# valette/FROG

Hardware: AMD Instinct MI355X
Metric: registration iterations/sec (linear+deformable) (higher is better)
Workload: dtype f32

## Files before the change

frog_amd/_abi.py:

```python
import ctypes as C
import os

_HERE = os.path.dirname(os.path.abspath(__file__))
LIB_DIR = os.path.join(_HERE, "lib")



def usable_cpus():
    import math
    n = len(os.sched_getaffinity(0)) if hasattr(os, "sched_getaffinity") else (os.cpu_count() or 1)

    def quota(d):
        try:
            with open(os.path.join(d, "cpu.max")) as fh:
                q, p = fh.read().split()[:2]
            return None if q == "max" else float(q) / float(p)
        except (OSError, ValueError):
            pass
        try:
            with open(os.path.join(d, "cpu.cfs_quota_us")) as fh:
                q = float(fh.read())
            with open(os.path.join(d, "cpu.cfs_period_us")) as fh:
                p = float(fh.read())
            return q / p if q > 0 and p > 0 else None
# ... 322 lines not shown
    "frog_labels_fused": (C.c_int, [C.c_void_p, C.POINTER(FrogVolume), c_float_p]),
    "frog_labels_probability": (C.c_int, [C.c_void_p, C.c_int64, c_float_p]),
    "frog_labels_destroy": (None, [C.c_void_p]),
    "frog_staple_create": (C.c_int, [C.POINTER(FrogVolume), C.c_uint32, C.c_uint32, C.c_int, C.POINTER(C.c_void_p)]),
    "frog_staple_add": (C.c_int, [C.c_void_p, C.c_void_p, C.POINTER(FrogVolume), C.c_double, C.POINTER(FrogVolume)]),
    "frog_staple_finish": (C.c_int, [C.c_void_p, c_u32_p]),
    "frog_staple_values": (C.c_int, [C.c_void_p, C.POINTER(C.c_int64)]),
    "frog_staple_solve": (C.c_int, [C.c_void_p, C.c_double, C.c_double, C.c_uint32, C.c_int, c_u32_p, c_double_p,
                                    C.POINTER(C.c_uint64)]),
    "frog_staple_fused": (C.c_int, [C.c_void_p, C.POINTER(FrogVolume), c_float_p]),
    "frog_staple_probability": (C.c_int, [C.c_void_p, C.c_int64, c_float_p]),
    "frog_staple_performance": (C.c_int, [C.c_void_p, c_double_p, C.POINTER(C.c_uint64), C.POINTER(C.c_uint64), c_double_p]),
    "frog_staple_destroy": (None, [C.c_void_p]),
    "frog_wlabels_create": (C.c_int, [C.POINTER(FrogVolume), C.c_uint32, C.c_uint32, C.c_uint32, C.c_uint32, C.c_float, C.c_int,
                                      C.POINTER(C.c_void_p)]),
    "frog_wlabels_target": (C.c_int, [C.c_void_p, C.c_void_p, C.POINTER(FrogVolume), C.c_int, C.c_double, C.POINTER(FrogVolume)]),
    "frog_wlabels_add": (C.c_int, [C.c_void_p, C.c_void_p, C.POINTER(FrogVolume), C.POINTER(FrogVolume), C.c_int, C.c_double,
                                   C.c_double, C.POINTER(FrogVolume), C.POINTER(FrogVolume)]),
    "frog_wlabels_finish": (C.c_int, [C.c_void_p, c_u32_p]),
    "frog_wlabels_values": (C.c_int, [C.c_void_p, C.POINTER(C.c_int64)]),
    "frog_wlabels_fused": (C.c_int, [C.c_void_p, C.c_int64, C.POINTER(FrogVolume), c_float_p]),
    "frog_wlabels_probability": (C.c_int, [C.c_void_p, C.c_int64, c_float_p]),
    "frog_wlabels_destroy": (None, [C.c_void_p]),
    "frog_jlabels_create": (C.c_int, [C.POINTER(FrogVolume), C.c_uint32, C.c_uint32, C.c_uint32, C.c_uint32, C.c_double, C.c_int, C.c_int,
                                      C.POINTER(C.c_void_p)]),
    "frog_jlabels_target": (C.c_int, [C.c_void_p, C.c_void_p, C.POINTER(FrogVolume), C.c_int, C.c_double, C.POINTER(FrogVolume)]),
    "frog_jlabels_add": (C.c_int, [C.c_void_p, C.c_void_p, C.POINTER(FrogVolume), C.POINTER(FrogVolume), C.c_int, C.c_double,
                                   C.c_double, C.POINTER(FrogVolume), C.POINTER(FrogVolume)]),
    "frog_jlabels_finish": (C.c_int, [C.c_void_p, c_u32_p]),
    "frog_jlabels_values": (C.c_int, [C.c_void_p, C.POINTER(C.c_int64)]),
    "frog_jlabels_fused": (C.c_int, [C.c_void_p, C.c_int64, C.POINTER(FrogVolume), c_float_p]),
    "frog_jlabels_probability": (C.c_int, [C.c_void_p, C.c_int64, c_float_p]),
    "frog_jlabels_weight": (C.c_int, [C.c_void_p, C.c_uint32, c_float_p]),
    "frog_jlabels_destroy": (None, [C.c_void_p]),
    "frog_distance_map": (C.c_int, [C.POINTER(FrogVolume), C.c_int64, C.c_int, C.c_int, c_u32_p]),
    "frog_surface_create": (C.c_int, [C.POINTER(FrogVolume), C.POINTER(C.c_int64), C.c_uint32, C.c_uint32, C.c_int,
                                      C.POINTER(C.c_void_p)]),
    "frog_surface_add": (C.c_int, [C.c_void_p, C.c_void_p, C.POINTER(FrogVolume), C.c_double, C.POINTER(FrogSurfaceRow)]),
    "frog_surface_destroy": (None, [C.c_void_p]),
    "frog_isosurface_create": (C.c_int, [C.POINTER(FrogVolume), C.c_int, C.c_double, C.c_int64, C.c_int, C.POINTER(C.c_void_p),
                                         c_u32_p, c_u32_p]),
    "frog_isosurface_apply": (C.c_int, [C.c_void_p, C.c_void_p]),
    "frog_isosurface_get": (C.c_int, [C.c_void_p, c_float_p, c_u32_p]),
    "frog_isosurface_destroy": (None, [C.c_void_p]),
    "frog_chain_apply_f32": (C.c_int, [C.c_void_p, c_float_p, c_float_p, C.c_size_t]),
    "frog_match_options_default": (None, [C.POINTER(FrogMatchOptions)]),
    "frog_matcher_create": (C.c_int, [C.POINTER(FrogKeypoints), C.c_uint32, C.c_int, C.POINTER(C.c_void_p)]),
    "frog_matcher_destroy": (None, [C.c_void_p]),
    "frog_matcher_run": (C.c_int, [C.c_void_p, C.POINTER(C.c_uint16), C.POINTER(C.c_uint16), C.c_size_t,
                                   C.POINTER(FrogMatchOptions), C.POINTER(C.c_uint64), C.POINTER(c_u32_p),
                                   C.POINTER(c_u32_p)]),
    "frog_match_free": (None, [C.c_void_p]),
    "frog_matcher_last_stats": (C.c_int, [C.c_void_p, c_double_p, c_double_p]),
    "frog_matcher_last_forms": (C.c_int, [C.c_void_p, C.POINTER(C.c_uint64)]),
    "frog_match_test_products": (C.c_int, [C.c_int, c_float_p, c_float_p, C.c_uint32, C.c_int, c_float_p, c_float_p]),
    "frog_get_points2_subset": (C.c_int, [C.c_void_p, C.POINTER(C.c_uint64), C.c_size_t, c_float_p]),
    "frog_set_hard_links": (C.c_int, [C.c_void_p, C.POINTER(C.c_uint64), C.POINTER(C.c_uint64), C.c_size_t, C.c_float]),
    "frog_residual_sums": (C.c_int, [C.c_void_p]),
    "frog_get_error_map": (C.c_int, [C.c_void_p, C.c_uint32, C.POINTER(FrogGridInfo), c_float_p, C.c_size_t]),
    "frog_comm_buffer": (C.c_int, [C.c_void_p, C.c_int, C.POINTER(C.c_void_p), C.POINTER(C.c_size_t),
                                   C.POINTER(C.c_size_t), C.POINTER(C.c_size_t)]),
    "frog_update_stats_local": (C.c_int, [C.c_void_p]),
    "frog_stats_publish": (C.c_int, [C.c_void_p]),
    "frog_transform_points_local": (C.c_int, [C.c_void_p, C.c_int]),
    "frog_linear_step_local": (C.c_int, [C.c_void_p]),
    "frog_energy_read": (C.c_int, [C.c_void_p, c_double_p, c_double_p]),
    "frog_bounds_local": (C.c_int, [C.c_void_p, c_double_p, c_double_p]),
    "frog_deformable_setup_bounds": (C.c_int, [C.c_void_p, C.c_int, c_double_p, c_double_p, C.POINTER(FrogGridInfo)]),
    "frog_deformable_phase_a": (C.c_int, [C.c_void_p, C.c_float]),
    "frog_deformable_phase_b": (C.c_int, [C.c_void_p]),
    "frog_deformable_phase_c": (C.c_int, [C.c_void_p, c_double_p]),
    "frog_get_stream": (C.c_int, [C.c_void_p, C.POINTER(C.c_void_p), C.POINTER(C.c_int)]),
    "frog_comm_unpack_slab": (C.c_int, [C.c_void_p, C.c_void_p, C.c_uint64, C.c_uint32, C.POINTER(C.c_uint64), C.c_uint32]),
    "frog_comm_mode": (C.c_int, [C.c_void_p, C.c_int]),
    "frog_create_seconds": (C.c_int, [C.c_void_p, c_double_p, C.POINTER(C.c_int)]),
    "frog_lattice_reallocations": (C.c_int, [C.c_void_p, C.POINTER(C.c_int)]),
    "frog_transform_points_slab": (C.c_int, [C.c_void_p, C.c_int, C.c_int, C.c_void_p, C.c_uint64, C.c_uint32]),
    "frog_comm_unpack_slab_step": (C.c_int, [C.c_void_p, C.c_void_p, C.c_uint64, C.c_uint32, C.POINTER(C.c_uint64), C.c_uint32, C.c_uint32]),
    "frog_step_finish": (C.c_int, [C.c_void_p, C.POINTER(C.c_double)]),
    "frog_step_speculate": (C.c_int, [C.c_void_p]),
    "frog_cull_stats": (C.c_int, [C.c_void_p, C.POINTER(C.c_uint64), C.POINTER(C.c_uint64), C.POINTER(C.c_uint64)]),
    "frog_cull_stats_linear": (C.c_int, [C.c_void_p, C.POINTER(C.c_uint64), C.POINTER(C.c_uint64), C.POINTER(C.c_uint64)]),
    "frog_test_stray_points": (C.c_int, [C.c_void_p, C.POINTER(C.c_uint64)]),
    "frog_test_cull_ranges": (C.c_int, [C.c_void_p, C.POINTER(C.c_uint64), C.POINTER(C.c_uint64)]),
    "frog_test_cull_steps": (C.c_int, [C.c_void_p, C.POINTER(C.c_uint64), C.POINTER(C.c_uint64)]),
    "frog_test_cull_readback": (C.c_int, [C.c_void_p, c_float_p, c_float_p, c_float_p, c_u32_p, c_float_p, c_u32_p]),
    "frog_test_em_refit": (C.c_int, [C.c_void_p, C.c_int]),
    "frog_test_ransac_candidates": (C.c_int, [C.POINTER(FrogModel), C.c_uint32, C.POINTER(FrogRansacOptions), c_double_p,
                                              C.POINTER(C.c_ubyte), C.c_size_t, C.POINTER(C.c_size_t)]),
    "frog_test_ransac_census": (C.c_int, [C.c_void_p, C.POINTER(FrogModel), C.c_uint32, c_double_p, C.c_size_t, C.c_float,
                                          c_u32_p]),
    "frog_test_inlier_probability": (C.c_int, [C.c_int, c_float_p, c_float_p, C.c_size_t, c_float_p, c_float_p]),
    "frog_test_inlier_weight_pair": (C.c_int, [C.c_int, c_float_p, c_float_p, C.c_float, c_float_p, C.c_size_t, c_float_p,
                                              C.POINTER(C.c_ubyte)]),
    "frog_test_bspline_weights": (C.c_int, [C.c_int, C.c_void_p, C.c_size_t, C.c_void_p]),
    "frog_profile_enable": (C.c_int, [C.c_void_p, C.c_int]),
    "frog_profile_read": (C.c_int, [C.c_void_p, C.POINTER(FrogKernelTime), C.c_int]),
}

HOST_SYMBOLS = {
    "frog_pairs_read": (C.c_void_p, [C.c_char_p, C.POINTER(C.c_int)]),
    "frog_pairs_write": (C.c_int, [C.c_void_p, C.c_char_p]),
    "frog_pairs_free": (None, [C.c_void_p]),
    "frog_pairs_model": (None, [C.c_void_p, C.POINTER(FrogModel)]),
    "frog_pairs_num_pairs": (C.c_uint64, [C.c_void_p]),
    "frog_pairs_num_points": (C.c_uint64, [C.c_void_p]),
    "frog_pairs_num_images": (C.c_uint32, [C.c_void_p]),
    "frog_pairs_num_blocks": (C.c_uint32, [C.c_void_p]),
    "frog_host_threads": (C.c_int, []),
    "frog_pairs_block": (C.c_int, [C.c_void_p, C.c_uint32, C.POINTER(C.c_uint16), C.POINTER(C.c_uint16),
                                   C.POINTER(C.c_uint32), C.POINTER(c_u32_p), C.POINTER(c_u32_p)]),
    "frog_pairs_from_arrays": (C.c_void_p, [C.c_uint32, c_u32_p, c_float_p, c_float_p, C.c_uint32,
                                            C.POINTER(C.c_uint16), C.POINTER(C.c_uint16),
                                            C.POINTER(C.c_uint64), c_u32_p, c_u32_p]),
    "frog_synth_defaults": (None, [C.POINTER(FrogSynthParams)]),
    "frog_synth_generate": (C.c_void_p, [C.POINTER(FrogSynthParams)]),
    "frog_pairs_append_points": (C.c_int, [C.c_void_p, C.c_uint32, c_float_p, C.c_uint32]),
    "frog_pairs_set_points": (C.c_int, [C.c_void_p, C.c_uint32, c_float_p]),
    "frog_volume_read": (C.c_void_p, [C.c_char_p, C.POINTER(C.c_int)]),
    "frog_volume_free": (None, [C.c_void_p]),
    "frog_volume_view": (None, [C.c_void_p, C.POINTER(FrogVolume)]),
    "frog_volume_range": (C.c_int, [C.POINTER(FrogVolume), c_double_p, c_double_p]),
    "frog_volume_write": (C.c_int, [C.c_char_p, C.POINTER(FrogVolume)]),
    "frog_bbox_grid": (C.c_int, [C.c_char_p, C.c_double, C.POINTER(FrogVolume)]),
    "frog_score_metrics_from": (C.c_int, [C.POINTER(FrogScoreSums), C.POINTER(C.c_uint64), C.c_uint32, C.POINTER(FrogScoreMetrics)]),
    "frog_keypoints_read": (C.c_void_p, [C.c_char_p, C.POINTER(C.c_int)]),
    "frog_keypoints_free": (None, [C.c_void_p]),
    "frog_keypoints_count": (C.c_uint32, [C.c_void_p]),
    "frog_keypoints_view": (None, [C.c_void_p, C.POINTER(FrogKeypoints)]),
    "frog_keypoints_select": (C.c_int, [C.c_void_p, c_u32_p, C.c_uint32]),
    "frog_keypoints_write": (C.c_int, [C.c_char_p, C.POINTER(FrogKeypoints)]),
    "frog_transform_read": (C.c_void_p, [C.c_char_p, C.POINTER(C.c_int)]),
    "frog_transform_free": (None, [C.c_void_p]),
    "frog_transform_num_links": (C.c_uint32, [C.c_void_p]),
    "frog_transform_links": (C.POINTER(FrogChainLink), [C.c_void_p]),
    "frog_volume_geometry": (C.c_int, [C.c_char_p, C.POINTER(C.c_uint32), c_double_p, c_double_p]),
    "frog_nifti_write": (C.c_int, [C.c_char_p, C.POINTER(C.c_uint32), c_double_p, c_double_p, C.c_uint32, c_float_p]),
    "frog_run_schedule": (C.c_int, [C.c_void_p, C.c_void_p, C.POINTER(FrogSchedulePlan), C.POINTER(FrogScheduleResult)]),
    "frog_mesh_read": (C.c_void_p, [C.c_char_p, C.POINTER(C.c_int)]),
    "frog_mesh_view": (None, [C.c_void_p, C.POINTER(FrogMesh)]),
    "frog_mesh_free": (None, [C.c_void_p]),
    "frog_mesh_write": (C.c_int, [C.c_char_p, C.POINTER(FrogMesh)]),
    "frog_mesh_last_error": (C.c_char_p, []),
}

COMM_SYMBOLS = {
    "frog_comm_create_rccl": (C.c_int, [C.c_int, C.POINTER(C.c_int), C.POINTER(C.c_void_p)]),
    "frog_comm_create_loopback": (C.c_int, [C.c_int, C.POINTER(C.c_void_p)]),
    "frog_comm_unique_id": (C.c_int, [C.POINTER(C.c_ubyte)]),
    "frog_comm_create_rank": (C.c_int, [C.c_int, C.c_int, C.POINTER(C.c_ubyte), C.c_int, C.POINTER(C.c_void_p)]),
    "frog_comm_create_shm": (C.c_int, [C.c_int, C.c_int, C.c_char_p, C.c_int, C.POINTER(C.c_void_p)]),
    "frog_comm_set_rows": (C.c_int, [C.c_void_p, C.POINTER(C.c_uint64)]),
    "frog_comm_destroy_all": (None, [C.c_int, C.POINTER(C.c_void_p)]),
    "frog_comm_bind": (C.c_int, [C.c_void_p, C.c_void_p, c_u32_p]),
    "frog_comm_all_gather_xyz2": (C.c_int, [C.c_void_p]),
    "frog_comm_slab": (C.c_int, [C.c_void_p, C.POINTER(C.c_void_p), C.POINTER(C.c_uint64)]),
    "frog_comm_all_gather_slab": (C.c_int, [C.c_void_p]),
    "frog_comm_gather_points": (C.c_int, [C.c_void_p, C.c_int, C.c_int, C.c_uint32]),
    "frog_comm_all_reduce": (C.c_int, [C.c_void_p, C.c_int]),
    "frog_comm_all_reduce_bounds": (C.c_int, [C.c_void_p, c_double_p, c_double_p]),
    "frog_comm_barrier": (C.c_int, [C.c_void_p]),
    "frog_comm_timing": (C.c_int, [C.c_void_p, C.c_int]),
    "frog_comm_timing_read": (C.c_int, [C.c_void_p, c_double_p, C.POINTER(C.c_uint64), C.POINTER(C.c_uint64)]),
}


# ... 53 lines not shown
```

frog_amd/csrc/device/frog_hip.hip:

```cpp

#include "ctx.h"
#include <hip/hip_ext.h>
#include "prep.h"
#include "k_links.hip.h"
#include "k_stats.hip.h"
#include "k_grid.hip.h"
#include "k_comm.hip.h"
#include "k_cull.hip.h"
#include "k_ransac.hip.h"
#include "k_reforder.hip.h"
#include "k_refchain.hip.h"
#include "similarity.h"

#include <atomic>
#include <chrono>
#include <cmath>
#include <cstdlib>
#include <cstring>
#include <random>
#include <limits>
#include <new>

namespace frog {
thread_local std::string g_last_error;
// ... 2421 lines not shown
}

int frog_test_inlier_probability(int device, const float em3[3], const float *d2, size_t n, float *fast, float *exact)
{
    if (!em3 || (n && (!d2 || !fast || !exact))) return fail(FROG_E_INVALID, "null argument");
    int ndev = 0;
    if (hipGetDeviceCount(&ndev) != hipSuccess || ndev < 1) return fail(FROG_E_NODEVICE, "no HIP device");
    if (device < 0 || device >= ndev) return fail(FROG_E_INVALID, "device index out of range");
    FROG_HIP_CHECK(hipSetDevice(device));
    if (!n) return FROG_OK;
    DevBuf<float> dd, df, de;
    FROG_HIP_CHECK(dd.alloc(n)); FROG_HIP_CHECK(df.alloc(n)); FROG_HIP_CHECK(de.alloc(n));
    FROG_HIP_CHECK(hipMemcpy(dd.p, d2, n * sizeof(float), hipMemcpyHostToDevice));
    test_probability_kernel<<<div_up(n, 256), 256>>>(make_float4(em3[0], em3[1], em3[2], 0.f), dd.p, n, df.p, de.p);
    FROG_HIP_CHECK(hipGetLastError());
    FROG_HIP_CHECK(hipMemcpy(fast, df.p, n * sizeof(float), hipMemcpyDeviceToHost));
    FROG_HIP_CHECK(hipMemcpy(exact, de.p, n * sizeof(float), hipMemcpyDeviceToHost));
    return FROG_OK;
}

__global__ void test_weight_pair_kernel(const float4 emA, const float4 emB, float threshold, const float *d2, size_t n, float *weight,
                                        unsigned char *form)
{
    const size_t i = (size_t)blockIdx.x * blockDim.x + threadIdx.x;
    if (i >= n) return;
    const float theta = threshold - THRESHOLD_BAND;
    const EmFast fA = em_fast_of(emA, theta);
    EmFast fB = em_fast_of(emB, theta);
    fB.lo = fmaxf(fB.lo, fA.lo); fB.hi = fminf(fB.hi, fA.hi);
    bool in_range;
    float w = inlier_weight_pair(d2[i], fA, fB, in_range);
    unsigned char f = 0;
    if (w < theta) f = 2;
    else if (!in_range) { w = fminf(inlier_probability(d2[i], em_derived_of(emA)), inlier_probability(d2[i], em_derived_of(emB))); f = 1; }
    weight[i] = w; form[i] = f;
}

int frog_test_inlier_weight_pair(int device, const float emA3[3], const float emB3[3], float threshold, const float *d2, size_t n,
                                 float *weight, unsigned char *form)
{
    if (!emA3 || !emB3 || (n && (!d2 || !weight || !form))) return fail(FROG_E_INVALID, "null argument");
    int ndev = 0;
    if (hipGetDeviceCount(&ndev) != hipSuccess || ndev < 1) return fail(FROG_E_NODEVICE, "no HIP device");
    if (device < 0 || device >= ndev) return fail(FROG_E_INVALID, "device index out of range");
    FROG_HIP_CHECK(hipSetDevice(device));
    if (!n) return FROG_OK;
    DevBuf<float> dd, dw; DevBuf<unsigned char> df;
    FROG_HIP_CHECK(dd.alloc(n)); FROG_HIP_CHECK(dw.alloc(n)); FROG_HIP_CHECK(df.alloc(n));
    FROG_HIP_CHECK(hipMemcpy(dd.p, d2, n * sizeof(float), hipMemcpyHostToDevice));
    test_weight_pair_kernel<<<div_up(n, 256), 256>>>(make_float4(emA3[0], emA3[1], emA3[2], 0.f), make_float4(emB3[0], emB3[1], emB3[2], 0.f),
                                                      threshold, dd.p, n, dw.p, df.p);
    FROG_HIP_CHECK(hipGetLastError());
    FROG_HIP_CHECK(hipMemcpy(weight, dw.p, n * sizeof(float), hipMemcpyDeviceToHost));
    FROG_HIP_CHECK(hipMemcpy(form, df.p, n, hipMemcpyDeviceToHost));
    return FROG_OK;
}

__global__ void test_weights_kernel(const double *f, size_t n, double *out)
{
    const size_t i = (size_t)blockIdx.x * blockDim.x + threadIdx.x;
    if (i >= n) return;
    double F[4];
    bspline_weights<double>(F, f[i]);
    for (int k = 0; k < 4; k++) out[4 * i + k] = F[k];
}

int frog_test_bspline_weights(int device, const double *f, size_t n, double *out4n)
{
    if (n && (!f || !out4n)) return fail(FROG_E_INVALID, "null argument");
    int ndev = 0;
    if (hipGetDeviceCount(&ndev) != hipSuccess || ndev < 1) return fail(FROG_E_NODEVICE, "no HIP device");
    if (device < 0 || device >= ndev) return fail(FROG_E_INVALID, "device index out of range");
    FROG_HIP_CHECK(hipSetDevice(device));
    if (!n) return FROG_OK;
    DevBuf<double> df, dw;
    FROG_HIP_CHECK(df.alloc(n)); FROG_HIP_CHECK(dw.alloc(4 * n));
    FROG_HIP_CHECK(hipMemcpy(df.p, f, n * sizeof(double), hipMemcpyHostToDevice));
    test_weights_kernel<<<div_up(n, 256), 256>>>(df.p, n, dw.p);
    FROG_HIP_CHECK(hipGetLastError());
    FROG_HIP_CHECK(hipMemcpy(out4n, dw.p, 4 * n * sizeof(double), hipMemcpyDeviceToHost));
    return FROG_OK;
}

int frog_test_cull_ranges(frog_ctx *ctx, uint64_t *ranges, uint64_t *with_election)
{
    CTX_GUARD(ctx);
    if (!ranges || !with_election) return fail(FROG_E_INVALID, "null output");
    *ranges = 0; *with_election = 0;
    if (ctx->cull_builds && ctx->act_cnt.n) {
        std::vector<uint32_t> h(ctx->act_cnt.n);
        FROG_HIP_CHECK(hipMemcpyAsync(h.data(), ctx->act_cnt.p, ctx->act_cnt.bytes(), hipMemcpyDeviceToHost, ctx->stream));
        FROG_HIP_CHECK(hipStreamSynchronize(ctx->stream));
        for (uint32_t v : h) {
            if (v & ~CULL_DUP_BIT) (*ranges)++;
            if (v & CULL_DUP_BIT) (*with_election)++;
        }
    }
    return FROG_OK;
}

int frog_test_cull_steps(frog_ctx *ctx, uint64_t *listed_steps, uint64_t *steps_with_election)
{
    CTX_GUARD(ctx);
    if (!listed_steps || !steps_with_election) return fail(FROG_E_INVALID, "null output");
    *listed_steps = 0; *steps_with_election = 0;
    if (ctx->cull_builds && ctx->act_cnt.n) {
        std::vector<uint32_t> h(ctx->act_cnt.n), bits(ctx->act_steps.n);
        FROG_HIP_CHECK(hipMemcpyAsync(h.data(), ctx->act_cnt.p, ctx->act_cnt.bytes(), hipMemcpyDeviceToHost, ctx->stream));
        FROG_HIP_CHECK(hipMemcpyAsync(bits.data(), ctx->act_steps.p, ctx->act_steps.bytes(), hipMemcpyDeviceToHost, ctx->stream));
        FROG_HIP_CHECK(hipStreamSynchronize(ctx->stream));
        for (uint32_t v : h) *listed_steps += ((v & ~CULL_DUP_BIT) + 63u) / 64u;
        for (uint32_t v : bits) *steps_with_election += (uint64_t)__builtin_popcount(v);
    }
    return FROG_OK;
}

int frog_test_cull_readback(frog_ctx *ctx, float *cut_now, float *cut_list, float *allow, uint32_t *state, float *disp_max, uint32_t *disp_n)
{
    CTX_GUARD(ctx);
    if (!ctx->cut_now.p || !ctx->cut_list.p || !ctx->disp_part.p || !ctx->cull_state.p || !ctx->disp_allow.p)
        return fail(FROG_E_STATE, "the context has no culling list (FROG_CULL=0, a threshold below 1e-3, or its buffers did not fit)");
    hipStream_t s = ctx->stream;
    const uint32_t n = (uint32_t)std::min<size_t>(ctx->disp_n, ctx->disp_part.n);
    std::vector<uint32_t> part(disp_max ? n : 0);
    if (cut_now) FROG_HIP_CHECK(hipMemcpyAsync(cut_now, ctx->cut_now.p, (size_t)ctx->nI * sizeof(float), hipMemcpyDeviceToHost, s));
    if (cut_list) FROG_HIP_CHECK(hipMemcpyAsync(cut_list, ctx->cut_list.p, (size_t)ctx->nI * sizeof(float), hipMemcpyDeviceToHost, s));
    if (allow) FROG_HIP_CHECK(hipMemcpyAsync(allow, ctx->disp_allow.p, sizeof(float), hipMemcpyDeviceToHost, s));
    if (state) FROG_HIP_CHECK(hipMemcpyAsync(state, ctx->cull_state.p, sizeof(uint32_t), hipMemcpyDeviceToHost, s));
    if (!part.empty()) FROG_HIP_CHECK(hipMemcpyAsync(part.data(), ctx->disp_part.p, part.size() * sizeof(uint32_t), hipMemcpyDeviceToHost, s));
    FROG_HIP_CHECK(hipStreamSynchronize(s));
    if (disp_max) {
        uint32_t m = 0;
        for (uint32_t v : part) m = std::max(m, v);
        std::memcpy(disp_max, &m, sizeof m);
    }
    if (disp_n) *disp_n = n;
    return FROG_OK;
}

int frog_test_stray_points(frog_ctx *ctx, uint64_t *n)
{
    CTX_GUARD(ctx);
    { const int rc_ = join_setup(ctx); if (rc_) return rc_; }
    if (!n) return fail(FROG_E_INVALID, "null output");
    unsigned int v = 0;
    FROG_HIP_CHECK(hipMemcpyAsync(&v, ctx->stray.p + 2, sizeof v, hipMemcpyDeviceToHost, ctx->stream));
    FROG_HIP_CHECK(hipStreamSynchronize(ctx->stream));
    *n = v;
    return FROG_OK;
}

int frog_test_em_refit(frog_ctx *ctx, int term_by_term)
{
    CTX_GUARD(ctx);
    const uint32_t nO = ctx->n_owned(), cap = (uint32_t)ctx->sample_cap;
    const int cur = ctx->sel_used;
    hipStream_t s = ctx->stream;
    if (term_by_term)
        em_kernel<<<nO, 256, 0, s>>>(ctx->samples.p, ctx->sample_count[cur].p, cap, ctx->ib, ctx->em.p,
                                     ctx->opt.stats_max_iterations, ctx->opt.stats_epsilon);
    else
        em_scan_kernel<<<nO, EM_THREADS, 0, s>>>(ctx->samples.p, ctx->sample_count[cur].p, cap, ctx->ib, ctx->em.p,
                                                 ctx->opt.stats_max_iterations, ctx->opt.stats_epsilon, nullptr);
    FROG_HIP_CHECK(hipGetLastError());
    return frog_stats_publish(ctx);
}
// ... 187 lines not shown
```

frog_amd/csrc/device/k_grid.hip.h:

```cpp
#pragma once

#include "ctx.h"

namespace frog {

struct GeomDev {
    int dims[3];
    int n_cp;
    double origin[3];
    double spacing[3];
    double inv_spacing[3];
    int brick;
    int nbricks[3];
    int n_bricks;
    int lat_sh;
    uint32_t lat_mask;
    size_t lat_blk, lat_img;
    uint32_t mask_words;
};

__device__ __forceinline__ bool lat_active(const uint32_t *mask, const GeomDev &g, uint32_t img, uint32_t node)
{
    return (mask[(size_t)img * g.mask_words + (node >> 5)] >> (node & 31u)) & 1u;
}
// ... 738 lines not shown
        o.z = (float)((double)in[2] + (double)disp[2] * 1.0);
        o.w = v.w;
        pos2[p] = P3{ o.x, o.y, o.z };
        if (apply) pos[p] = o;
        if (snap) {
            const P3 q = snap[p];
            const float ex = o.x - q.x, ey = o.y - q.y, ez = o.z - q.z;
            dmax = max(dmax, __float_as_uint(__builtin_sqrtf(ex * ex + ey * ey + ez * ez)) & 0x7FFFFFFFu);
        }
    }
    if (snap) {
        #pragma unroll
        for (int off = 32; off > 0; off >>= 1) dmax = max(dmax, (uint32_t)__shfl_xor((int)dmax, off, 64));
        if (lane == 0) {
            disp_part[bid] = dmax;
            if (!(__uint_as_float(dmax) <= *disp_allow)) atomicOr(cull_state, 1u);
        }
    }
}

#ifdef FROG_SCATTER_TRACE
__device__ unsigned long long g_scatter_trace[4 * 65536];
#endif
constexpr int BRICK_CP_MAX = 11;


struct ScatterEnergy {
    const double *partial;
    uint32_t n;
    double *block_sums;
    unsigned int *ticket;
    double *energy;
    const uint32_t *list_invalid;
    unsigned int *stray_next;
    unsigned int *stray_total;
};

__device__ __forceinline__ void scatter_energy_block(const ScatterEnergy &en, const uint32_t r, const int lane)
{
    const uint32_t per = (en.n + ENERGY_BLOCKS - 1) / ENERGY_BLOCKS;
    const uint32_t b = min(en.n, r * per), e = min(en.n, b + per);
    double a0 = 0, a1 = 0;
    for (uint32_t t = b + lane; t < e; t += 64) { a0 += en.partial[2 * (size_t)t]; a1 += en.partial[2 * (size_t)t + 1]; }
    #pragma unroll
    for (int off = 32; off > 0; off >>= 1) { a0 += __shfl_down(a0, off, 64); a1 += __shfl_down(a1, off, 64); }
    bool last = false;
    if (lane == 0) {
        __hip_atomic_store(&en.block_sums[2 * r], a0, __ATOMIC_RELAXED, __HIP_MEMORY_SCOPE_AGENT);
        __hip_atomic_store(&en.block_sums[2 * r + 1], a1, __ATOMIC_RELAXED, __HIP_MEMORY_SCOPE_AGENT);
        __threadfence();
        last = atomicAdd(en.ticket, 1u) == (unsigned int)ENERGY_BLOCKS - 1u;
    }
    if (!__builtin_amdgcn_readfirstlane((int)last)) return;
    __threadfence();
    const double v0 = __hip_atomic_load(&en.block_sums[lane], __ATOMIC_RELAXED, __HIP_MEMORY_SCOPE_AGENT);
    const double v1 = __hip_atomic_load(&en.block_sums[64 + lane], __ATOMIC_RELAXED, __HIP_MEMORY_SCOPE_AGENT);
    double s0 = 0, s1 = 0;
    #pragma unroll 1
    for (int k = 0; k < ENERGY_BLOCKS; k++) {
        const int i0 = 2 * k, i1 = 2 * k + 1;
        const double x = __shfl(i0 < 64 ? v0 : v1, i0 & 63, 64), y = __shfl(i1 < 64 ? v0 : v1, i1 & 63, 64);
        s0 += x; s1 += y;
    }
    if (lane == 0) {
        en.energy[0] = s0; en.energy[1] = s1; en.energy[2] = 0.0;
        en.energy[3] = en.list_invalid ? (double)en.list_invalid[0] : 0.0;
        *en.stray_next = 0u;
        *en.ticket = 0u;
    }
}

#ifndef FROG_SCATTER_QUADS
#define FROG_SCATTER_QUADS 1
#endif
constexpr int SC_AHEAD = 3, SC_RING = 4;
#if FROG_SCATTER_QUADS
constexpr int SC_PTS = 64 + 4;
#else
constexpr int SC_PTS = 64 + SC_AHEAD;
#endif
struct ScatterScratch {
    float wx[4][SC_PTS], wy[4][SC_PTS];
    float wz[4][SC_PTS];
    float4 sm[SC_PTS];
    int base[SC_PTS];
};
static_assert(offsetof(ScatterScratch, sm) % 16 == 0, "ScatterScratch::sm is read with ds_read_b128");

#define FROG_FMAC_DPP(D, S, Q) "v_fmac_f32_dpp %" #D ", %" #S ", %8 quad_perm:[" #Q "," #Q "," #Q "," #Q "] row_mask:0xf bank_mask:0xf\n\t"
#define FROG_FMAC4_DPP(Q) asm volatile("s_nop 1\n\t" FROG_FMAC_DPP(0, 4, Q) FROG_FMAC_DPP(1, 5, Q) FROG_FMAC_DPP(2, 6, Q) FROG_FMAC_DPP(3, 7, Q)      \
                              : "+v"(run.x), "+v"(run.y), "+v"(run.z), "+v"(run.w) : "v"(s.x), "v"(s.y), "v"(s.z), "v"(s.w), "v"(w))
template <int P> __device__ __forceinline__ void fmac4_quad_bcast(float4 &run, const float4 s, float w)
{
    static_assert(P >= 0 && P < 4, "quad lane");
    if constexpr (P == 0) FROG_FMAC4_DPP(0);
    if constexpr (P == 1) FROG_FMAC4_DPP(1);
    if constexpr (P == 2) FROG_FMAC4_DPP(2);
    if constexpr (P == 3) FROG_FMAC4_DPP(3);
}

__global__ __launch_bounds__(64) void scatter_kernel(const float4 *pos_b, const float4 *point_sums,
                                                     const float4 *group_sums, uint32_t own_points, uint32_t own_pt_begin,
                                                     const uint32_t *perm, const ScatterBlock *blocks, const uint32_t *n_blocks,
                                                     float4 *gradf, float4 *stage, unsigned int *stray, const GeomDev g,
                                                     const ScatterEnergy en)
{
    if (en.partial && blockIdx.x < (uint32_t)ENERGY_BLOCKS) {
        scatter_energy_block(en, blockIdx.x, threadIdx.x);
        return;
    }
    const uint32_t bid = blockIdx.x - (en.partial ? (uint32_t)ENERGY_BLOCKS : 0u);
#ifdef FROG_SCATTER_TRACE
    const unsigned long long trace_t0 = wall_clock64();
    unsigned tr_load = 0, tr_p1 = 0, tr_p2 = 0;
#endif
    const ScatterBlock blk = blocks[bid];
    if (bid >= *n_blocks) return;
    extern __shared__ float4 tile[];
    __shared__ ScatterScratch sc;
    const int lane = threadIdx.x;
    const int E = g.brick + 3;
    const int n_tile = E * E * E;

    const uint32_t s_last = blk.end - 1u;
    const auto load_index = [&](uint32_t s) -> uint32_t { return perm[min(s, s_last)]; };
    const auto load_point = [&](uint32_t p, uint32_t s, float4 (&part)[N_XCD], float4 &v) __attribute__((always_inline)) {
        if (group_sums) {
            const uint32_t li = p - own_pt_begin;
            #pragma unroll
            for (int q = 0; q < N_XCD; q++) part[q] = group_sums[group_sum_index(q, li, own_points)];
        } else {
            part[0] = point_sums[p];
        }
        v = pos_b[min(s, s_last)];
    };
    uint32_t p_cur = load_index(blk.begin + lane);
    uint32_t p_nxt = load_index(blk.begin + 64 + lane);
    float4 part_cur[N_XCD], v_cur;
    #pragma unroll
    for (int q = 1; q < N_XCD; q++) part_cur[q] = make_float4(0.f, 0.f, 0.f, 0.f);
    load_point(p_cur, blk.begin + lane, part_cur, v_cur);

    for (int k = lane; k < n_tile; k += 64) tile[k] = make_float4(0.f, 0.f, 0.f, 0.f);

    const uint32_t img = blk.key / g.n_bricks;
    uint32_t bidx = blk.key - img * g.n_bricks;
    const int bx = bidx % g.nbricks[0]; bidx /= g.nbricks[0];
    const int by = bidx % g.nbricks[1];
    const int bz = bidx / g.nbricks[1];
    const int cp0[3] = { bx * g.brick, by * g.brick, bz * g.brick };

    const int ti = lane & 3, tj = (lane >> 2) & 3, tk = lane >> 4;
    const int tap_off = ti + E * (tj + E * tk);
    __builtin_amdgcn_fence(__ATOMIC_RELEASE, "wavefront");
    __builtin_amdgcn_wave_barrier();

    float4 run = make_float4(0.f, 0.f, 0.f, 0.f);
    int run_base = -1;
    for (uint32_t batch = blk.begin; batch < blk.end; batch += 64) {
        const uint32_t p_far = load_index(batch + 128 + lane);
        float4 part_nxt[N_XCD], v_nxt;
        #pragma unroll
        for (int q = 1; q < N_XCD; q++) part_nxt[q] = make_float4(0.f, 0.f, 0.f, 0.f);
        load_point(p_nxt, batch + 64 + lane, part_nxt, v_nxt);
#ifdef FROG_SCATTER_TRACE
        const unsigned long long tb0 = wall_clock64();
        asm volatile("s_waitcnt vmcnt(10)" ::: "memory");
        const unsigned long long tb1 = wall_clock64();
#endif
        float wxy[16], wz[4], wx4[4], wy4[4];
        float4 sm = part_cur[0];
        int base = -1;
        if (batch + lane < blk.end) {
            if (group_sums) {
                #pragma unroll
                for (int q = 1; q < N_XCD; q++) { sm.x += part_cur[q].x; sm.y += part_cur[q].y; sm.z += part_cur[q].z; sm.w += part_cur[q].w; }
            }
            if (sm.w != 0.f) {
                const float in[3] = { v_cur.x, v_cur.y, v_cur.z };
                int ic[3]; float fr[3];
                scatter_cell(in, g, ic, fr);
                double F[4];
                float w12[12];
                #pragma unroll
                for (int ax = 0; ax < 3; ax++) {
                    bspline_weights(F, (double)fr[ax]);
                    #pragma unroll
                    for (int m = 0; m < 4; m++) w12[ax * 4 + m] = (float)F[m];
                }
                #pragma unroll
                for (int j = 0; j < 4; j++)
                    #pragma unroll
                    for (int i = 0; i < 4; i++) wxy[4 * j + i] = w12[i] * w12[4 + j];
                #pragma unroll
                for (int k = 0; k < 4; k++) { wz[k] = w12[8 + k]; wx4[k] = w12[k]; wy4[k] = w12[4 + k]; }
                const int lx = ic[0] - 1 - cp0[0], ly = ic[1] - 1 - cp0[1], lz = ic[2] - 1 - cp0[2];
                if (lx >= 0 && ly >= 0 && lz >= 0 && lx + 3 < E && ly + 3 < E && lz + 3 < E) {
                    base = lx + E * (ly + E * lz);
                } else {
                    atomicAdd(stray, 1u);
                    atomicAdd(en.stray_total, 1u);
                    for (int k = 0; k < 4; k++) for (int j = 0; j < 4; j++) for (int i = 0; i < 4; i++) {
                        const int gx = ic[0] - 1 + i, gy = ic[1] - 1 + j, gz = ic[2] - 1 + k;
                        if (gx < 0 || gy < 0 || gz < 0 || gx >= g.dims[0] || gy >= g.dims[1] || gz >= g.dims[2]) continue;
                        const float w = wxy[4 * j + i] * wz[k];
                        float *dst = reinterpret_cast<float *>(gradf + lat(g, img, (uint32_t)gx + (uint32_t)g.dims[0] * ((uint32_t)gy + (uint32_t)g.dims[1] * (uint32_t)gz)));
                        atomicAdd(dst + 0, w * sm.x); atomicAdd(dst + 1, w * sm.y);
                        atomicAdd(dst + 2, w * sm.z); atomicAdd(dst + 3, w * sm.w);
                    }
                }
            }
        }
        const unsigned long long live = __ballot(base >= 0);
        const int n_live = __popcll(live);
        if (base >= 0) {
            const int slot = __popcll(live & ((1ull << lane) - 1ull));
            #pragma unroll
            for (int k = 0; k < 4; k++) { sc.wx[k][slot] = wx4[k]; sc.wy[k][slot] = wy4[k]; }
            #pragma unroll
            for (int k = 0; k < 4; k++) sc.wz[k][slot] = wz[k];
            sc.sm[slot] = sm;
            sc.base[slot] = base;
        }
        __builtin_amdgcn_fence(__ATOMIC_RELEASE, "wavefront");
        __builtin_amdgcn_wave_barrier();
#ifdef FROG_SCATTER_TRACE
        const unsigned long long tb2 = wall_clock64();
#endif

        unsigned long long chg;
        {
            const int mine = lane < n_live ? sc.base[lane] : -1;
            const int before = lane == 0 ? run_base : (lane < n_live ? sc.base[lane - 1] : -1);
            chg = __ballot(lane < n_live && mine != before);
        }
#if FROG_SCATTER_QUADS
        {
            const f32x4 *gwx = reinterpret_cast<const f32x4 *>(sc.wx[lane & 3]), *gwy = reinterpret_cast<const f32x4 *>(sc.wy[(lane >> 2) & 3]),
                        *gwz = reinterpret_cast<const f32x4 *>(sc.wz[lane >> 4]);
            const float4 *gsm = sc.sm + (lane & 3);
            f32x4 cwx = gwx[0], cwy = gwy[0], cwz = gwz[0];
            float4 csm4 = gsm[0];
            auto spill_and_restart = [&](int q) __attribute__((always_inline)) {
                if (run_base >= 0) {
                    float4 t = tile[run_base + tap_off];
                    t.x += run.x; t.y += run.y; t.z += run.z; t.w += run.w;
                    tile[run_base + tap_off] = t;
                }
                run = make_float4(0.f, 0.f, 0.f, 0.f);
                run_base = __builtin_amdgcn_readfirstlane(sc.base[q]);
            };
            for (int q0 = 0; q0 < n_live; q0 += 4) {
                const int g1 = (q0 >> 2) + 1;
                const f32x4 nwx = gwx[g1], nwy = gwy[g1], nwz = gwz[g1];
                const float4 nsm = gsm[4 * g1];
                const f32x4 w4 = (cwx * cwy) * cwz;
                const unsigned m = (unsigned)(chg >> q0) & 15u;
                const int left = n_live - q0;
#define FROG_SCATTER_ADD(P)                                                                                            \
                if (P < left) {                                                                                         \
                    if (m >> P & 1u) spill_and_restart(q0 + P);                                                         \
                    fmac4_quad_bcast<P>(run, csm4, w4[P]);                                                              \
                }
                FROG_SCATTER_ADD(0) FROG_SCATTER_ADD(1) FROG_SCATTER_ADD(2) FROG_SCATTER_ADD(3)
#undef FROG_SCATTER_ADD
                cwx = nwx; cwy = nwy; cwz = nwz; csm4 = nsm;
            }
        }
#else
        float rwx[SC_RING], rwz[SC_RING];
        float4 rsm[SC_RING];
        float rwy[SC_RING];
        const float *lane_wx = sc.wx[lane & 3], *lane_wy = sc.wy[(lane >> 2) & 3], *lane_wz = sc.wz[lane >> 4];
        auto fetch = [&](int q, int slot) __attribute__((always_inline)) {
            rwx[slot] = lane_wx[q];
            rwy[slot] = lane_wy[q];
            rwz[slot] = lane_wz[q];
            rsm[slot] = sc.sm[q];
        };
        auto add_point = [&](int q, int slot) __attribute__((always_inline)) {
            if ((chg >> q) & 1ull) {
                if (run_base >= 0) {
                    float4 t = tile[run_base + tap_off];
                    t.x += run.x; t.y += run.y; t.z += run.z; t.w += run.w;
                    tile[run_base + tap_off] = t;
                }
                run = make_float4(0.f, 0.f, 0.f, 0.f);
                run_base = __builtin_amdgcn_readfirstlane(sc.base[q]);
            }
            const float w = (rwx[slot] * rwy[slot]) * rwz[slot];
            const float4 csm = rsm[slot];
            run.x = fmaf(w, csm.x, run.x); run.y = fmaf(w, csm.y, run.y); run.z = fmaf(w, csm.z, run.z); run.w = fmaf(w, csm.w, run.w);
        };
        #pragma unroll
        for (int j = 0; j < SC_AHEAD; j++) fetch(j, j);
        const int n_full = n_live & ~(SC_RING - 1);
        for (int q0 = 0; q0 < n_full; q0 += SC_RING) {
            #pragma unroll
            for (int j = 0; j < SC_RING; j++) {
                fetch(q0 + j + SC_AHEAD, (j + SC_AHEAD) % SC_RING);
                add_point(q0 + j, j);
            }
        }
        #pragma unroll
        for (int j = 0; j < SC_RING - 1; j++)
            if (n_full + j < n_live) add_point(n_full + j, j);
#endif
        __builtin_amdgcn_fence(__ATOMIC_RELEASE, "wavefront");
        __builtin_amdgcn_wave_barrier();
#ifdef FROG_SCATTER_TRACE
        {
            const unsigned long long tb3 = wall_clock64();
            tr_load += __builtin_amdgcn_readfirstlane((unsigned)(tb1 - tb0));
            tr_p1 += __builtin_amdgcn_readfirstlane((unsigned)(tb2 - tb1));
            tr_p2 += __builtin_amdgcn_readfirstlane((unsigned)(tb3 - tb2));
        }
#endif
        p_cur = p_nxt; p_nxt = p_far; v_cur = v_nxt;
        #pragma unroll
        for (int q = 0; q < N_XCD; q++) part_cur[q] = part_nxt[q];
    }
    if (run_base >= 0) {
        float4 t = tile[run_base + tap_off];
        t.x += run.x; t.y += run.y; t.z += run.z; t.w += run.w;
        tile[run_base + tap_off] = t;
    }
    __builtin_amdgcn_fence(__ATOMIC_RELEASE, "wavefront");
    __builtin_amdgcn_wave_barrier();

    float4 *dst = stage + (size_t)blk.slot * n_tile;
    for (int k = lane; k < n_tile; k += 64) dst[k] = tile[k];
#ifdef FROG_SCATTER_TRACE
    if (lane == 0 && bid < 65536) {
        unsigned int hw, xcc;
        asm volatile("s_getreg_b32 %0, hwreg(HW_REG_HW_ID)" : "=s"(hw));
        asm volatile("s_getreg_b32 %0, hwreg(HW_REG_XCC_ID)" : "=s"(xcc));
        g_scatter_trace[4 * bid + 0] = trace_t0;
        g_scatter_trace[4 * bid + 1] = wall_clock64();
        g_scatter_trace[4 * bid + 2] = ((unsigned long long)xcc << 32) | hw;
        g_scatter_trace[4 * bid + 3] = (unsigned long long)(blk.end - blk.begin) | ((unsigned long long)(tr_load & 0xFFFF) << 16)
                                              | ((unsigned long long)(tr_p1 & 0xFFFF) << 32) | ((unsigned long long)(tr_p2 & 0xFFFF) << 48);
    }
#endif
}

constexpr int LS_CPB = 16;
constexpr int LS_IC = 64;
constexpr int LS_THREADS = LS_CPB * LS_IC;
constexpr int LS_CPB_SMALL = 4;
constexpr int LS_SMALL_NODES = 2048;
constexpr int LS_KEEP = 8;
static_assert(LS_THREADS <= 1024 && 3 * LS_CPB <= LS_THREADS, "lattice_step_kernel thread mapping");

struct LatticeStepArgs {
    const float4 *stage;
    const uint32_t *brick_slot_ptr;
    float4 *gradf;
    unsigned int *stray;
    const float4 *coeff;
    float4 *grad;
    double *gridsum;
    double *energy_tail;
    uint32_t n_owned, n_images;
    float alpha;
    double lim[3];
    double *energy;
    const uint32_t *mask;
    const uint32_t *n_inactive;
    const float4 *ucoeff;
    float4 *ugrad;
// ... 293 lines not shown
```

include/frog_hip.h:

```cpp
#ifndef FROG_HIP_H
#define FROG_HIP_H

#include "frog_types.h"

#ifdef __cplusplus
extern "C" {
#endif

typedef struct frog_ctx frog_ctx;


int frog_device_count(void);
int frog_device_warm(int device);
const char *frog_last_error(void);

int frog_create(const frog_model *model, const frog_options *options, int device,
                uint32_t image_begin, uint32_t image_end, frog_ctx **out);
void frog_destroy(frog_ctx *ctx);

int frog_set_stream(frog_ctx *ctx, void *hip_stream);
int frog_create_seconds(frog_ctx *ctx, double seconds3[3], int *selections_replayed);
int frog_lattice_reallocations(frog_ctx *ctx, int *count);

int frog_get_stream(frog_ctx *ctx, void **hip_stream, int *device);
// ... 7 lines not shown

typedef struct frog_ransac_options {
    int32_t iterations;
    int32_t batches;
    float   inlier_distance;
    float   max_scale;
} frog_ransac_options;
int frog_ransac(frog_ctx *ctx, const frog_model *model, uint32_t image, const frog_ransac_options *options,
                int64_t *n_inliers);
int frog_deformable_setup(frog_ctx *ctx, int level, frog_grid_info *out);
int frog_deformable_step(frog_ctx *ctx, float alpha, double *E);
int frog_count_inliers(frog_ctx *ctx, frog_counts *per_image);


uint64_t frog_num_points(const frog_ctx *ctx);
uint32_t frog_num_images(const frog_ctx *ctx);
int frog_get_points(frog_ctx *ctx, float *xyz, float *xyz2);
int frog_set_points2(frog_ctx *ctx, const float *xyz2);
int frog_get_points2_subset(frog_ctx *ctx, const uint64_t *points, size_t n, float *xyz2_out3n);
int frog_get_linear(frog_ctx *ctx, uint32_t image, double matrix16[16]);
int frog_get_em(frog_ctx *ctx, uint32_t image, float c1_c2_ratio[3]);
int frog_set_em(frog_ctx *ctx, uint32_t image, const float c1_c2_ratio[3]);
int frog_set_em_rows(frog_ctx *ctx, const float *table4, uint32_t image_begin, uint32_t image_end);
int frog_get_samples(frog_ctx *ctx, uint32_t image, float *samples, uint32_t *ordinals,
                     int cap, int *n);
int frog_get_histogram(frog_ctx *ctx, uint32_t image, float *bins, int cap, int *n);
int frog_num_grids(const frog_ctx *ctx);
int frog_get_grid(frog_ctx *ctx, uint32_t image, int k, frog_grid_info *info,
                  float *coeffs, size_t cap_floats);
int frog_get_point_sums(frog_ctx *ctx, float *out4P);
int frog_get_gradient(frog_ctx *ctx, uint32_t image, float *out4G, size_t cap_floats);

int frog_set_hard_links(frog_ctx *ctx, const uint64_t *point, const uint64_t *partner, size_t n, float weight2);

int frog_residual_sums(frog_ctx *ctx);
int frog_get_error_map(frog_ctx *ctx, uint32_t image, frog_grid_info *info, float *out4G, size_t cap_floats);


enum {
    FROG_BUF_XYZ2    = 0,
    FROG_BUF_EM      = 1,
    FROG_BUF_ENERGY  = 2,
    FROG_BUF_GRIDSUM = 3
};
int frog_comm_buffer(frog_ctx *ctx, int which, void **device_ptr, size_t *bytes,
                     size_t *row_begin, size_t *row_end);

int frog_comm_unpack_slab(frog_ctx *ctx, const void *slab, uint64_t slot_rows, uint32_t world_size,
                          const uint64_t *row_begin, uint32_t self);

#define FROG_SLAB_TRAILER_BYTES 64
#define FROG_SLAB_SLOT_BYTES(slot_rows) (((size_t)(slot_rows) * 12 + 63) / 64 * 64 + FROG_SLAB_TRAILER_BYTES)
int frog_comm_mode(frog_ctx *ctx, int two_collectives);
int frog_transform_points_slab(frog_ctx *ctx, int apply, int after_step, void *slab, uint64_t slot_rows, uint32_t self);
int frog_comm_unpack_slab_step(frog_ctx *ctx, const void *slab, uint64_t slot_rows, uint32_t world_size,
                               const uint64_t *row_begin, uint32_t self, uint32_t sum_mask);
int frog_step_finish(frog_ctx *ctx, double *E);
int frog_step_speculate(frog_ctx *ctx);

int frog_update_stats_local(frog_ctx *ctx);
int frog_stats_publish(frog_ctx *ctx);
int frog_transform_points_local(frog_ctx *ctx, int apply);
int frog_linear_step_local(frog_ctx *ctx);
int frog_energy_read(frog_ctx *ctx, double *E, double *n_oversize);
int frog_bounds_local(frog_ctx *ctx, double mins[3], double maxs[3]);
int frog_deformable_setup_bounds(frog_ctx *ctx, int level, const double mins[3],
                                 const double maxs[3], frog_grid_info *out);
int frog_deformable_phase_a(frog_ctx *ctx, float alpha);
int frog_deformable_phase_b(frog_ctx *ctx);
int frog_deformable_phase_c(frog_ctx *ctx, double *E);

int frog_cull_stats(frog_ctx *ctx, uint64_t *lists_built, uint64_t *listed_half_links, uint64_t *owned_half_links);
int frog_cull_stats_linear(frog_ctx *ctx, uint64_t *lists_built, uint64_t *listed_half_links, uint64_t *owned_half_links);

int frog_test_inlier_probability(int device, const float c1_c2_ratio[3], const float *d2, size_t n,
                                 float *fast, float *exact);

int frog_test_inlier_weight_pair(int device, const float c1_c2_ratio_a[3], const float c1_c2_ratio_b[3], float inlier_threshold,
                                 const float *d2, size_t n, float *weight, unsigned char *form);

int frog_test_bspline_weights(int device, const double *f, size_t n, double *out4n);

int frog_test_stray_points(frog_ctx *ctx, uint64_t *n);
int frog_test_cull_ranges(frog_ctx *ctx, uint64_t *ranges, uint64_t *with_election);
int frog_test_cull_steps(frog_ctx *ctx, uint64_t *listed_steps, uint64_t *steps_with_election);
int frog_test_cull_readback(frog_ctx *ctx, float *cut_now, float *cut_list, float *allow, uint32_t *state, float *disp_max,
                            uint32_t *disp_n);

int frog_test_ransac_candidates(const frog_model *model, uint32_t image, const frog_ransac_options *options, double *cand12n,
                                unsigned char *usable, size_t cap, size_t *n);
int frog_test_ransac_census(frog_ctx *ctx, const frog_model *model, uint32_t image, const double *cand12n, size_t n,
                            float inlier_distance, uint32_t *counts);

int frog_test_em_refit(frog_ctx *ctx, int term_by_term);

enum {
    FROG_K_SWEEP_LINEAR = 0,
    FROG_K_SWEEP_DEFORMABLE,
    FROG_K_SCATTER,
    FROG_K_LATTICE,
    FROG_K_TRANSFORM,
    FROG_K_STATS,
    FROG_K_COMBINE,
    FROG_K_CULL,
    FROG_K_SWEEP_BUILD,
    FROG_K_SWEEP_LINEAR_BUILD,
    FROG_K_COUNT_
};
typedef struct frog_kernel_time {
    double   ms_total;
    uint64_t launches;
} frog_kernel_time;
int frog_profile_enable(frog_ctx *ctx, int on);
int frog_profile_read(frog_ctx *ctx, frog_kernel_time *out, int reset);

#ifdef __cplusplus
}
#endif
#endif
```

Before: 2520.

## Accumulate scatter contributions with 4x4x1 MFMA instead of DPP fmac broadcasts

```diff
diff --git a/frog_amd/_abi.py b/frog_amd/_abi.py
--- a/frog_amd/_abi.py
+++ b/frog_amd/_abi.py
@@ -428,6 +428,7 @@
     "frog_cull_stats": (C.c_int, [C.c_void_p, C.POINTER(C.c_uint64), C.POINTER(C.c_uint64), C.POINTER(C.c_uint64)]),
     "frog_cull_stats_linear": (C.c_int, [C.c_void_p, C.POINTER(C.c_uint64), C.POINTER(C.c_uint64), C.POINTER(C.c_uint64)]),
     "frog_test_stray_points": (C.c_int, [C.c_void_p, C.POINTER(C.c_uint64)]),
+    "frog_test_scatter_accumulate": (C.c_int, [C.c_int, c_float_p, c_float_p, C.c_size_t, c_float_p, c_float_p, C.c_int]),
     "frog_test_cull_ranges": (C.c_int, [C.c_void_p, C.POINTER(C.c_uint64), C.POINTER(C.c_uint64)]),
     "frog_test_cull_steps": (C.c_int, [C.c_void_p, C.POINTER(C.c_uint64), C.POINTER(C.c_uint64)]),
     "frog_test_cull_readback": (C.c_int, [C.c_void_p, c_float_p, c_float_p, c_float_p, c_u32_p, c_float_p, c_u32_p]),
diff --git a/frog_amd/csrc/device/frog_hip.hip b/frog_amd/csrc/device/frog_hip.hip
--- a/frog_amd/csrc/device/frog_hip.hip
+++ b/frog_amd/csrc/device/frog_hip.hip
@@ -2527,6 +2527,46 @@
     return FROG_OK;
 }
 
+__global__ __launch_bounds__(64, 4) void test_scatter_accumulate_kernel(const float *sums, const float *weights, uint32_t n, const float *start,
+                                                                     float *out, int plain)
+{
+    const int lane = threadIdx.x;
+    f32x4 run = { start[4 * lane], start[4 * lane + 1], start[4 * lane + 2], start[4 * lane + 3] };
+    for (uint32_t q = 0; q < n; q++) {
+        const float w = weights[64 * (size_t)q + lane];
+        if (plain) {
+            #pragma unroll
+            for (int c = 0; c < 4; c++) run[c] = fmaf(w, sums[4 * (size_t)q + c], run[c]);
+        } else {
+            scatter_accumulate(run, sums[4 * (size_t)q + (lane & 3)], w);
+        }
+    }
+    #pragma unroll
+    for (int c = 0; c < 4; c++) out[4 * lane + c] = run[c];
+}
+
+int frog_test_scatter_accumulate(int device, const float *sums4n, const float *weights64n, size_t n, const float *start256, float *out256,
+                                 int plain)
+{
+    if (!start256 || !out256 || (n && (!sums4n || !weights64n))) return fail(FROG_E_INVALID, "null argument");
+    if (n > (1u << 20)) return fail(FROG_E_INVALID, "too many points");
+    int ndev = 0;
+    if (hipGetDeviceCount(&ndev) != hipSuccess || ndev < 1) return fail(FROG_E_NODEVICE, "no HIP device");
+    if (device < 0 || device >= ndev) return fail(FROG_E_INVALID, "device index out of range");
+    FROG_HIP_CHECK(hipSetDevice(device));
+    DevBuf<float> ds, dw, d0, d1;
+    FROG_HIP_CHECK(ds.alloc(4 * n + 1)); FROG_HIP_CHECK(dw.alloc(64 * n + 1)); FROG_HIP_CHECK(d0.alloc(256)); FROG_HIP_CHECK(d1.alloc(256));
+    if (n) {
+        FROG_HIP_CHECK(hipMemcpy(ds.p, sums4n, 4 * n * sizeof(float), hipMemcpyHostToDevice));
+        FROG_HIP_CHECK(hipMemcpy(dw.p, weights64n, 64 * n * sizeof(float), hipMemcpyHostToDevice));
+    }
+    FROG_HIP_CHECK(hipMemcpy(d0.p, start256, 256 * sizeof(float), hipMemcpyHostToDevice));
+    test_scatter_accumulate_kernel<<<1, 64>>>(ds.p, dw.p, (uint32_t)n, d0.p, d1.p, plain);
+    FROG_HIP_CHECK(hipGetLastError());
+    FROG_HIP_CHECK(hipMemcpy(out256, d1.p, 256 * sizeof(float), hipMemcpyDeviceToHost));
+    return FROG_OK;
+}
+
 int frog_test_cull_ranges(frog_ctx *ctx, uint64_t *ranges, uint64_t *with_election)
 {
     CTX_GUARD(ctx);
diff --git a/frog_amd/csrc/device/k_grid.hip.h b/frog_amd/csrc/device/k_grid.hip.h
--- a/frog_amd/csrc/device/k_grid.hip.h
+++ b/frog_amd/csrc/device/k_grid.hip.h
@@ -844,24 +844,19 @@
 struct ScatterScratch {
     float wx[4][SC_PTS], wy[4][SC_PTS];
     float wz[4][SC_PTS];
-    float4 sm[SC_PTS];
+    float sm[4][SC_PTS];
     int base[SC_PTS];
 };
-static_assert(offsetof(ScatterScratch, sm) % 16 == 0, "ScatterScratch::sm is read with ds_read_b128");
-
-#define FROG_FMAC_DPP(D, S, Q) "v_fmac_f32_dpp %" #D ", %" #S ", %8 quad_perm:[" #Q "," #Q "," #Q "," #Q "] row_mask:0xf bank_mask:0xf\n\t"
-#define FROG_FMAC4_DPP(Q) asm volatile("s_nop 1\n\t" FROG_FMAC_DPP(0, 4, Q) FROG_FMAC_DPP(1, 5, Q) FROG_FMAC_DPP(2, 6, Q) FROG_FMAC_DPP(3, 7, Q)      \
-                              : "+v"(run.x), "+v"(run.y), "+v"(run.z), "+v"(run.w) : "v"(s.x), "v"(s.y), "v"(s.z), "v"(s.w), "v"(w))
-template <int P> __device__ __forceinline__ void fmac4_quad_bcast(float4 &run, const float4 s, float w)
-{
-    static_assert(P >= 0 && P < 4, "quad lane");
-    if constexpr (P == 0) FROG_FMAC4_DPP(0);
-    if constexpr (P == 1) FROG_FMAC4_DPP(1);
-    if constexpr (P == 2) FROG_FMAC4_DPP(2);
-    if constexpr (P == 3) FROG_FMAC4_DPP(3);
-}
-
-__global__ __launch_bounds__(64) void scatter_kernel(const float4 *pos_b, const float4 *point_sums,
+#if FROG_SCATTER_QUADS
+static_assert(offsetof(ScatterScratch, sm) % 16 == 0 && SC_PTS % 4 == 0, "the rows of ScatterScratch are read with ds_read_b128");
+#endif
+
+__device__ __forceinline__ void scatter_accumulate(f32x4 &run, const float s_comp, const float w)
+{
+    run = __builtin_amdgcn_mfma_f32_4x4x1f32(s_comp, w, run, 0, 0, 0);
+}
+
+__global__ __launch_bounds__(64, 4) void scatter_kernel(const float4 *pos_b, const float4 *point_sums,
                                                      const float4 *group_sums, uint32_t own_points, uint32_t own_pt_begin,
                                                      const uint32_t *perm, const ScatterBlock *blocks, const uint32_t *n_blocks,
                                                      float4 *gradf, float4 *stage, unsigned int *stray, const GeomDev g,
@@ -917,7 +912,7 @@
     __builtin_amdgcn_fence(__ATOMIC_RELEASE, "wavefront");
     __builtin_amdgcn_wave_barrier();
 
-    float4 run = make_float4(0.f, 0.f, 0.f, 0.f);
+    f32x4 run = { 0.f, 0.f, 0.f, 0.f };
     int run_base = -1;
     for (uint32_t batch = blk.begin; batch < blk.end; batch += 64) {
         const uint32_t p_far = load_index(batch + 128 + lane);
@@ -981,7 +976,7 @@
             for (int k = 0; k < 4; k++) { sc.wx[k][slot] = wx4[k]; sc.wy[k][slot] = wy4[k]; }
             #pragma unroll
             for (int k = 0; k < 4; k++) sc.wz[k][slot] = wz[k];
-            sc.sm[slot] = sm;
+            sc.sm[0][slot] = sm.x; sc.sm[1][slot] = sm.y; sc.sm[2][slot] = sm.z; sc.sm[3][slot] = sm.w;
             sc.base[slot] = base;
         }
         __builtin_amdgcn_fence(__ATOMIC_RELEASE, "wavefront");
@@ -1000,33 +995,36 @@
         {
             const f32x4 *gwx = reinterpret_cast<const f32x4 *>(sc.wx[lane & 3]), *gwy = reinterpret_cast<const f32x4 *>(sc.wy[(lane >> 2) & 3]),
                         *gwz = reinterpret_cast<const f32x4 *>(sc.wz[lane >> 4]);
-            const float4 *gsm = sc.sm + (lane & 3);
-            f32x4 cwx = gwx[0], cwy = gwy[0], cwz = gwz[0];
-            float4 csm4 = gsm[0];
+            const f32x4 *gsm = reinterpret_cast<const f32x4 *>(sc.sm[lane & 3]);
             auto spill_and_restart = [&](int q) __attribute__((always_inline)) {
                 if (run_base >= 0) {
                     float4 t = tile[run_base + tap_off];
                     t.x += run.x; t.y += run.y; t.z += run.z; t.w += run.w;
                     tile[run_base + tap_off] = t;
                 }
-                run = make_float4(0.f, 0.f, 0.f, 0.f);
+                run = f32x4{ 0.f, 0.f, 0.f, 0.f };
                 run_base = __builtin_amdgcn_readfirstlane(sc.base[q]);
             };
-            for (int q0 = 0; q0 < n_live; q0 += 4) {
-                const int g1 = (q0 >> 2) + 1;
-                const f32x4 nwx = gwx[g1], nwy = gwy[g1], nwz = gwz[g1];
-                const float4 nsm = gsm[4 * g1];
-                const f32x4 w4 = (cwx * cwy) * cwz;
+            auto add_group = [&](const int q0, const f32x4 wx, const f32x4 wy, const f32x4 wz, const f32x4 sm4) __attribute__((always_inline)) {
+                const f32x4 w4 = (wx * wy) * wz;
                 const unsigned m = (unsigned)(chg >> q0) & 15u;
                 const int left = n_live - q0;
-#define FROG_SCATTER_ADD(P)                                                                                            \
+#define FROG_SCATTER_ADD(P)                                                                                           \
                 if (P < left) {                                                                                         \
                     if (m >> P & 1u) spill_and_restart(q0 + P);                                                         \
-                    fmac4_quad_bcast<P>(run, csm4, w4[P]);                                                              \
+                    scatter_accumulate(run, sm4[P], w4[P]);                                                             \
                 }
                 FROG_SCATTER_ADD(0) FROG_SCATTER_ADD(1) FROG_SCATTER_ADD(2) FROG_SCATTER_ADD(3)
 #undef FROG_SCATTER_ADD
-                cwx = nwx; cwy = nwy; cwz = nwz; csm4 = nsm;
+            };
+            f32x4 awx = gwx[0], awy = gwy[0], awz = gwz[0], asm4 = gsm[0];
+            for (int q0 = 0; q0 < n_live; q0 += 8) {
+                const int g1 = (q0 >> 2) + 1;
+                const f32x4 bwx = gwx[g1], bwy = gwy[g1], bwz = gwz[g1], bsm4 = gsm[g1];
+                add_group(q0, awx, awy, awz, asm4);
+                if (q0 + 4 >= n_live) break;
+                awx = gwx[g1 + 1]; awy = gwy[g1 + 1]; awz = gwz[g1 + 1]; asm4 = gsm[g1 + 1];
+                add_group(q0 + 4, bwx, bwy, bwz, bsm4);
             }
         }
 #else
@@ -1038,7 +1036,7 @@
             rwx[slot] = lane_wx[q];
             rwy[slot] = lane_wy[q];
             rwz[slot] = lane_wz[q];
-            rsm[slot] = sc.sm[q];
+            rsm[slot] = make_float4(sc.sm[0][q], sc.sm[1][q], sc.sm[2][q], sc.sm[3][q]);
         };
         auto add_point = [&](int q, int slot) __attribute__((always_inline)) {
             if ((chg >> q) & 1ull) {
@@ -1047,7 +1045,7 @@
                     t.x += run.x; t.y += run.y; t.z += run.z; t.w += run.w;
                     tile[run_base + tap_off] = t;
                 }
-                run = make_float4(0.f, 0.f, 0.f, 0.f);
+                run = f32x4{ 0.f, 0.f, 0.f, 0.f };
                 run_base = __builtin_amdgcn_readfirstlane(sc.base[q]);
             }
             const float w = (rwx[slot] * rwy[slot]) * rwz[slot];
diff --git a/include/frog_hip.h b/include/frog_hip.h
--- a/include/frog_hip.h
+++ b/include/frog_hip.h
@@ -113,6 +113,8 @@
 int frog_test_bspline_weights(int device, const double *f, size_t n, double *out4n);
 
 int frog_test_stray_points(frog_ctx *ctx, uint64_t *n);
+int frog_test_scatter_accumulate(int device, const float *sums4n, const float *weights64n, size_t n, const float *start256,
+                                 float *out256, int plain);
 int frog_test_cull_ranges(frog_ctx *ctx, uint64_t *ranges, uint64_t *with_election);
 int frog_test_cull_steps(frog_ctx *ctx, uint64_t *listed_steps, uint64_t *steps_with_election);
 int frog_test_cull_readback(frog_ctx *ctx, float *cut_now, float *cut_list, float *allow, uint32_t *state, float *disp_max,
```

Result: faster. 2565 (median of 6 runs) (+1.8%).
